# MecatronicaUSB/uw-slam

Hardware: AMD Instinct MI355X
Metric: frame-pair alignments/sec (640x480, 4 pyr lvls) (higher is better)
Workload: dtype f32; 1 GPU; synthetic 640x480 pairs, 4 pyramid levels (0..3), 10 GN iterations/level, no early exit, dense points, u16 depth plane, 1024 pairs in total, 1024 resident on rank 0 (128 distinct), image pyramids of both frames + depth pyramid and gradients of the reference frame + alignment per step; normal_equation_accumulation=f64, weights=identity, tuning=defaults, sampler=nearest, total_pairs=1024, pairs_on_rank0=1024

## Files before the change

uw-slam_amd/csrc/uwt_capi.hip:

```cpp
#include "uwt_ctx.h"

namespace {

constexpr int kGroupsPerThread = 1;

uwt_tuning default_tuning() {
  uwt_tuning t;
  std::memset(&t, 0, sizeof(t));
  t.split = 2;
  t.split_min = 8;
  t.split_min_px = 32LL * 640 * 480;
  t.stream_bytes = 200LL << 20;
  t.tail_update = 1;
  t.target_blocks = 0;
  t.coarse = 1;
  t.coarse_batch_px = kCoarseMaxPixels;
  t.coarse_weighted = 1;
  t.overlap_gradients = 1;
  t.first_poll = 3;
  t.chained = -1;
  t.speculation = 1;
  t.fused_stages = 1;
  t.pyramid_batch = 1;
  t.typed_loads = 1;
// ... 333 lines not shown
  };
  int smax = 1;
  for (int lvl = p.first_level; lvl >= p.last_level; lvl--) {
    int gpb, sl;
    level_slicing(c, lvl, n_pairs, target_blocks, !p.early_exit, gpb, sl);
    smax = std::max(smax, sl);
  }
  if (general && p.weights)
    HIPCHK(c, hipMemsetAsync(c->hist, 0, sizeof(unsigned int) * kHistBins * n_pairs, c->stream));
  bool coarse_lvl[UWT_MAX_LEVELS] = {};
  if (p.accumulate_f64 != 0 && (!general || (p.sampler == 0 && p.weights != 0 && c->tn.coarse_weighted)) && c->tn.coarse_batch_px > 0 &&
      !c->compute_only && !(c->profiling && p.early_exit))
    for (int lvl = p.first_level; lvl >= p.last_level; lvl--)
      coarse_lvl[lvl] = c->lv[lvl].ng <= c->tn.coarse_batch_px;
  auto run_coarse = [&](int base, int cnt, hipStream_t s, int lvl, bool resume) -> int {
    CoarseArgs ca = coarse_args(update_rule(p, general), start.rec(p), InlinePairs{});
    coarse_level(c, ca, 0, lvl);
    ca.n_levels = 1;
    ca.u.pair_base = base;
    ca.state_out = c->state;
    ca.resume = resume ? 1 : 0;
    size_t ev = 0;
    if (c->profiling) {
      int st = prof_begin(c, &ev, lvl, p.max_iters);
      if (st) return st;
    }
    uwt::launch_coarse_level(s, launch_sel(c), ca, cnt, general ? p.weights : 0);
    HIPCHK(c, hipGetLastError());
    if (c->profiling) HIPCHK(c, prof_end(c, ev, s, (long long)cnt * c->lv[lvl].gw * c->lv[lvl].gh, p.max_iters));
    return UWT_OK;
  };
  const bool tickets = c->tn.tail_update >= (parts > 1 ? 1 : 2);
  const bool tail = tickets && !c->compute_only;
  if (tickets) HIPCHK(c, hipMemsetAsync(c->d_tickets, 0, sizeof(unsigned int) * (size_t)n_pairs, c->stream));
  struct Part { int base, cnt; hipStream_t s; ResidualArgs ra; UpdateArgs ua; };
  Part pt[uwt_ctx::kMaxParts];
  const bool window = opt.window && !general && !p.early_exit && p.last_level == 0 && p.first_level >= 1 && !c->profiling &&
                      !c->compute_only;
  struct JoinGuard {
    uwt_ctx* c; int parts; bool joined = false;
    ~JoinGuard() {
      if (joined) return;
      for (int i = 1; i < parts; i++) (void)hipStreamSynchronize(c->part_stream[i]);
    }
  } guard{c, parts};
  if (parts > 1) HIPCHK(c, hipEventRecord(c->ev_fork, c->stream));
  for (int i = 0; i < parts; i++) {
    Part& q = pt[i];
    q.base = (int)((long long)n_pairs * i / parts);
    q.cnt = (int)((long long)n_pairs * (i + 1) / parts) - q.base;
    q.s = i ? c->part_stream[i] : c->stream;
    if (i) HIPCHK(c, hipStreamWaitEvent(q.s, c->ev_fork, 0));
    if (!coarse_lvl[p.first_level]) {
      hipLaunchKernelGGL(k_init_state, dim3((q.cnt + tb - 1) / tb), dim3(tb), 0, q.s, c->state + q.base, q.cnt, start.rec(p, q.base),
                         nullptr);
      HIPCHK(c, hipGetLastError());
    }
  }
  for (int lvl = p.first_level; lvl >= p.last_level; lvl--) {
    for (int i = 0; i < parts; i++) {
      Part& q = pt[i];
      HIPCHK(c, wait_level(c, q.s, level_ready, lvl));
      if (coarse_lvl[lvl]) {
        int st = run_coarse(q.base, q.cnt, q.s, lvl, lvl != p.first_level);
        if (st) return st;
        if (window && lvl == 1) HIPCHK(c, hipEventRecord(c->ev_window[i], q.s));
        continue;
      }
      q.ra = residual_args(c, lvl);
      q.ua = update_args(c, lvl, general);
      q.ra.pair_base = q.ua.pair_base = q.base;
      q.ra.stream_planes = streams(lvl);
      level_slicing(c, lvl, n_pairs, target_blocks, !p.early_exit, q.ra.groups_per_block, q.ra.slices);
      q.ua.slices = q.ra.slices;
      const size_t shift = (size_t)q.base * (size_t)(smax - q.ra.slices) * kRecWords;
      q.ra.partials = c->partials + shift;
      q.ua.partials = c->partials + shift;
    }
    if (coarse_lvl[lvl]) continue;
    LatePoll late(c->tn.first_poll);
    bool level_done = false;
    for (int k = 0; k < p.max_iters && !level_done; k++)
      for (int i = 0; i < parts; i++) {
        Part& q = pt[i];
        size_t ev = 0;
        if (c->profiling) {
          int st = prof_begin(c, &ev, lvl);
          if (st) return st;
          q.ra.probe = 1;
          c->prof_slices = q.ra.slices;
          c->prof_pairs = q.cnt;
          c->prof_records = c->partials;
        }
        q.ua.k = k;
        int st = late.arm(c, q.s, p.early_exit != 0, k, p.max_iters, &q.ua.active);
        if (st) return st;
        if (tail) arm_tail(c, q.ra, q.ua);
        st = general ? launch_general(c, q.s, q.ra, q.cnt, false) : launch_residual(c, q.s, q.ra, q.cnt, false);
        if (st) return st;
        if (c->profiling) HIPCHK(c, prof_end(c, ev, q.s, (long long)q.cnt * c->lv[lvl].gw * c->lv[lvl].gh));
        if (!tail) {
          hipLaunchKernelGGL(k_gn_update, dim3(q.cnt), dim3(kUpdateBlock), 0, q.s, q.ua);
          HIPCHK(c, hipGetLastError());
        }
        st = late.look(c, q.s, &level_done);
        if (st) return st;
        if (level_done) break;
      }
    for (int i = 0; i < parts; i++) {
      hipLaunchKernelGGL(k_level_end, dim3((pt[i].cnt + tb - 1) / tb), dim3(tb), 0, pt[i].s, c->state + pt[i].base, pt[i].cnt, lvl,
                         start.rec(p));
      HIPCHK(c, hipGetLastError());
      if (window && lvl == 1) HIPCHK(c, hipEventRecord(c->ev_window[i], pt[i].s));
    }
  }
  for (int i = 0; i < parts; i++) {
    hipLaunchKernelGGL(k_write_out, dim3((pt[i].cnt + tb - 1) / tb), dim3(tb), 0, pt[i].s, c->state + pt[i].base, pt[i].cnt,
                       d_poses + 7 * (size_t)pt[i].base, d_stats ? d_stats + pt[i].base : nullptr);
    HIPCHK(c, hipGetLastError());
    if (window && parts > 1 && i == 0) HIPCHK(c, hipEventRecord(c->ev_first_end, pt[0].s));
    if (i) {
      HIPCHK(c, hipEventRecord(c->ev_join[i], pt[i].s));
      HIPCHK(c, hipStreamWaitEvent(c->stream, c->ev_join[i], 0));
    }
  }
  guard.joined = true;
  if (window) c->win_parts = parts;
  return UWT_OK;
}

int dep_note(uwt_ctx* c, uwt_ctx::SlotDep* ring, int& next, bool& dropped, hipStream_t on, int first, int n) {
  uwt_ctx::SlotDep& d = ring[next];
  if (d.used) dropped = true;
  d.first = first; d.n = n; d.used = true;
  HIPCHK(c, hipEventRecord(d.ev, on));
  next = (next + 1) % uwt_ctx::kDeps;
  return UWT_OK;
}

}

namespace uwt {

int first_failure(uwt_ctx* c, const char* what, const uwt_stats* stats, int n) {
  for (int i = 0; i < n; i++)
    if (stats[i].status != UWT_OK)
      return fail(c, UWT_ERR_PAIR_FAILED, std::string(what) + ": at least one pair failed, first status: " +
                                              uwt_status_string(stats[i].status));
  return UWT_OK;
}

int seed_options(uwt_ctx* c, const char* what, const uwt_seed_options* sopt, Start* out) {
  *out = Start();
  if (!sopt) return UWT_OK;
  if (sopt->handoff < 0 || sopt->handoff > 1)
    return fail(c, UWT_ERR_INVALID_ARG, std::string(what) + ": uwt_seed_options: handoff outside 0..1");
  for (int32_t r : sopt->reserved)
    if (r) return fail(c, UWT_ERR_INVALID_ARG, std::string(what) + ": uwt_seed_options: reserved word not zero");
  out->keep = sopt->handoff;
  return UWT_OK;
// ... 590 lines not shown
  for (hipEvent_t e : {c->ev_fork, c->ev_pyramids, c->ev_side_done, c->ev_entry, c->ev_first_end}) drop(e);
  for (int i = 0; i < uwt_ctx::kDeps; i++) { drop(c->busy[i].ev); drop(c->fresh[i].ev); }
  for (hipStream_t s : c->part_stream)
    if (s) (void)hipStreamDestroy(s);
  for (hipStream_t s : {c->side, c->copy, c->stream})
    if (s) (void)hipStreamDestroy(s);
  delete c;
  return UWT_OK;
}

int uwt_get_params(const uwt_ctx* c, uwt_params* out) {
  if (!c || !out) return UWT_ERR_INVALID_ARG;
  *out = c->p;
  return UWT_OK;
}

int uwt_get_tuning(const uwt_ctx* c, uwt_tuning* out) {
  if (!c || !out) return UWT_ERR_INVALID_ARG;
  *out = c->tn;
  return UWT_OK;
}

int uwt_set_tuning(uwt_ctx* c, const uwt_tuning* t) {
  if (!c || !t) return UWT_ERR_INVALID_ARG;
  if (t->split < 1 || t->split > uwt_ctx::kMaxParts || t->split_min < 1 || t->split_min_px < 1 || t->stream_bytes < 0 ||
      t->tail_update < 0 || t->tail_update > 2 || t->target_blocks < 0 || t->target_blocks > (1 << 20) || t->coarse_batch_px < 0 ||
      t->coarse_batch_px > (1 << 24) || t->first_poll < 1 || t->first_poll > (1 << 20) || t->chained < -1 || t->chained > 1)
    return fail(c, UWT_ERR_INVALID_ARG, "uwt_set_tuning: value out of range");
  (void)hipSetDevice(c->p.device);
  close_window(c);
  HIPCHK(c, hipStreamSynchronize(c->stream));
  HIPCHK(c, hipStreamSynchronize(c->side));
  c->tn = *t;
  c->spec_budget = c->spec_calm = 0;
  for (int32_t* b : {&c->tn.coarse, &c->tn.coarse_weighted, &c->tn.speculation, &c->tn.fused_stages, &c->tn.pyramid_batch, &c->tn.typed_loads})
    *b = *b != 0;
  if (c->tn.overlap_gradients < 0 || c->tn.overlap_gradients > 3) c->tn.overlap_gradients = 1;
  std::memset(c->tn.reserved, 0, sizeof(c->tn.reserved));
  return UWT_OK;
}

int uwt_update_params(uwt_ctx* c, const uwt_params* p) {
  if (!c || !p) return UWT_ERR_INVALID_ARG;
  const uwt_params& o = c->p;
  if (p->width != o.width || p->height != o.height || p->fx != o.fx || p->fy != o.fy || p->cx != o.cx || p->cy != o.cy ||
      p->n_levels != o.n_levels || p->has_depth != o.has_depth || p->max_frames != o.max_frames ||
      p->max_pairs != o.max_pairs || p->device != o.device || p->depth_scale != o.depth_scale)
    return fail(c, UWT_ERR_INVALID_ARG, "uwt_update_params: geometry / capacity fields differ from the context's");
  if (p->first_level >= p->n_levels || p->last_level < 0 || p->last_level > p->first_level || p->max_iters < 1 ||
      p->sampler < 0 || p->sampler > 1 || p->weights < 0 || p->weights > 2 || (p->sampler == 1 && p->weights == 1) ||
      (p->arith != UWT_ARITH_OPENCV && p->arith != UWT_ARITH_LEGACY))
    return fail(c, UWT_ERR_INVALID_ARG, "uwt_update_params: bad solver constants");
  (void)hipSetDevice(o.device);
  close_window(c);
  HIPCHK(c, hipStreamSynchronize(c->stream));
  if (p->sampler || p->weights) {
    const int st = ensure_general_buffers(c);
    if (st) return st;
  }
  c->p = *p;
  c->spec_budget = c->spec_calm = 0;
  return UWT_OK;
}

int uwt_level_info(const uwt_ctx* c, int32_t lvl, uwt_level* out) {
  if (!c || !out || lvl < 0 || lvl >= c->p.n_levels) return UWT_ERR_INVALID_ARG;
  *out = c->info[lvl];
  return UWT_OK;
}

int uwt_set_frame(uwt_ctx* c, int32_t slot, const uint8_t* gray, size_t row_stride, const uint16_t* depth,
                  size_t depth_row_stride) {
  if (c) (void)hipSetDevice(c->p.device);
  if (!c || !gray || !slot_range_ok(c, slot, 1)) return fail(c, UWT_ERR_INVALID_ARG, "uwt_set_frame: bad slot/pointer");
  const int w = c->p.width;
  if (row_stride < (size_t)w) return fail(c, UWT_ERR_INVALID_ARG, "uwt_set_frame: row stride < width");
  int st0 = compute_begin(c, slot, 1);
  if (st0) return st0;
  if (c->p.has_depth && (!depth || depth_row_stride < (size_t)w * 2)) return fail(c, UWT_ERR_INVALID_ARG, "uwt_set_frame: depth required");
  if ((st0 = copy_strided_frame_in(c, c->img[0], gray, 1, row_stride, slot, c->stream))) return st0;
  if (c->p.has_depth && (st0 = copy_strided_frame_in(c, c->depth[0], depth, 2, depth_row_stride, slot, c->stream))) return st0;
  HIPCHK(c, hipStreamSynchronize(c->stream));
  return UWT_OK;
}

int uwt_host_alloc(size_t bytes, void** out) {
  if (!out || !bytes) return UWT_ERR_INVALID_ARG;
  *out = nullptr;
  return hipHostMalloc(out, bytes) == hipSuccess ? UWT_OK : UWT_ERR_HIP;
}

int uwt_host_free(void* p) { return (!p || hipHostFree(p) == hipSuccess) ? UWT_OK : UWT_ERR_HIP; }

// ... 204 lines not shown
    const int base = c->tn.first_poll + 1;
    if (c->h_small->cut == 0) {
      if (c->spec_budget > base && ++c->spec_calm >= uwt_ctx::kSpecCalm) { c->spec_budget = std::max(base, c->spec_budget / 2); c->spec_calm = 0; }
      break;
    }
    c->spec_calm = 0;
    c->spec_budget = std::min(c->p.max_iters, 2 * std::max(c->spec_budget, base));
    if (attempt == 1) opt.speculate = false;
  }
  if (c->profiling) {
    st = prof_collect(c);
    if (st) return st;
  }
  if (stats_out) std::copy(tmp.begin(), tmp.end(), stats_out);
  return first_failure(c, what, tmp.data(), n_pairs);
}

int uwt_estimate_pose_batch(uwt_ctx* c, int32_t n_pairs, const int32_t* ref_slots, const int32_t* tgt_slots,
                            float* poses_out, uwt_stats* stats_out) {
  return estimate_pose_batch(c, "uwt_estimate_pose_batch", n_pairs, ref_slots, tgt_slots, poses_out, stats_out, nullptr, nullptr);
}

int uwt_default_seed_options(uwt_seed_options* o) {
  if (!o) return UWT_ERR_INVALID_ARG;
  std::memset(o, 0, sizeof(*o));
  return UWT_OK;
}

int uwt_estimate_pose_batch_seeded(uwt_ctx* c, int32_t n_pairs, const int32_t* ref_slots, const int32_t* tgt_slots,
                                   float* poses_out, uwt_stats* stats_out, const float* seeds, const uwt_seed_options* sopt) {
  return estimate_pose_batch(c, "uwt_estimate_pose_batch_seeded", n_pairs, ref_slots, tgt_slots, poses_out, stats_out, seeds, sopt);
}

static int track_batch_enqueue(uwt_ctx* c, int32_t first_slot, int32_t n_frames, int32_t grad_refs_only, int32_t n_pairs,
                               const int32_t* ref_slots, const int32_t* tgt_slots, float* d_poses_out, uwt_stats* d_stats_out,
                               const Start& start = Start()) {
  if (c) (void)hipSetDevice(c->p.device);
  if (!c) return fail(c, UWT_ERR_INVALID_ARG, "uwt_track_batch_async: bad argument");
  const bool had_window = c->win_open;
  const int win_parts = c->win_parts;
  close_window(c);
  c->win_parts = 0;
  if (!d_poses_out || !slot_range_ok(c, first_slot, n_frames))
    return fail(c, UWT_ERR_INVALID_ARG, "uwt_track_batch_async: bad argument");
  int st = seeds_clear_of(c, "uwt_track_batch_seeded_async", start.d_seeds, n_pairs, d_poses_out, d_stats_out);
  if (st) return st;
  const int og = c->tn.overlap_gradients;
  const bool overlap = og != 0 && !c->profiling && (n_pairs >= 768 || og == 3);
  const bool early = had_window && overlap && og != 2;
  st = check_pair_lists_range(c, n_pairs, ref_slots, tgt_slots);
  if (st) return st;
  struct SideGuard {
    uwt_ctx* c; bool armed = false;
    ~SideGuard() { if (armed) (void)hipStreamSynchronize(c->side); }
  } side_guard{c};
  if (early) {
    HIPCHK(c, hipEventRecord(c->ev_entry, c->stream));
    side_guard.armed = true;
    for (int i = 0; i < win_parts; i++) HIPCHK(c, hipStreamWaitEvent(c->side, c->ev_window[i], 0));
    if (win_parts > 1) HIPCHK(c, hipStreamWaitEvent(c->side, c->ev_first_end, 0));
  }
  st = send_pairs(c, n_pairs, ref_slots, tgt_slots, early);
  if (st) return st;
  int lo = first_slot, hi = first_slot + n_frames;
  for (int i = 0; i < n_pairs; i++) {
    lo = std::min(lo, std::min(ref_slots[i], tgt_slots[i]));
    hi = std::max(hi, std::max(ref_slots[i], tgt_slots[i]) + 1);
  }
  c->dep_first = lo;
// ... 171 lines not shown
```

uw-slam_amd/csrc/uwt_capi_tables.hip:

```cpp
#include "uwt_ctx.h"
#include "uwt_track.h"

extern "C" {

namespace {

int check_keypoints(uwt_ctx* c, const char* what, const float* kp, int n) {
  const float w = (float)c->lv[0].gw, h = (float)c->lv[0].gh;
  for (int i = 0; i < std::min(n, kPatchMaxKeypoints); i++)
    if (!inside_level0(kp[2 * i], kp[2 * i + 1], w, h))
      return fail(c, UWT_ERR_INVALID_ARG, std::string(what) + ": key point outside the image");
  return UWT_OK;
}

struct CandidatesLayout {
  int bands;
  size_t o_sums, o_mag, o_cells, o_off;
};
CandidatesLayout candidates_work_layout(Carve& cv, const LevelK& L, int n) {
  CandidatesLayout o;
  const int col_blocks = (L.gw + kBlock - 1) / kBlock;
  o.bands = std::max(1, std::min(L.gh / 8, 512 / std::max(1, col_blocks * n)));
  const size_t m = (size_t)L.gw * o.bands * n;
  o.o_sums = cv.take<unsigned long long>((size_t)n);
// ... 192 lines not shown
  HIPCHK(c, hipEventRecord(c->ev_feat[stage], c->stream));
  return enqueue_patch_producer(c, n, d_slots);
}

int table_options(uwt_ctx* c, const char* what, const uwt_table_options* opt, uwt_table_options* out) {
  std::memset(out, 0, sizeof(*out));
  if (!opt) return UWT_OK;
  if (opt->weights < 0 || opt->weights > 2 || opt->sampler < 0 || opt->sampler > 1)
    return fail(c, UWT_ERR_INVALID_ARG, std::string(what) + ": uwt_table_options: weights outside 0..2 or sampler outside 0..1");
  for (int32_t r : opt->reserved)
    if (r) return fail(c, UWT_ERR_INVALID_ARG, std::string(what) + ": uwt_table_options: reserved word not zero");
  *out = *opt;
  return UWT_OK;
}
constexpr uwt_table_options kIdentityTables = {};

struct TableLevel {
  TableArgs ta;
  int slices;
};

int enqueue_table_estimate(uwt_ctx* c, int n_pairs, const uwt_params& q, const TableLevel* lv, uint32_t* recs, bool polls,
                           const uwt_table_options& opt, float* d_poses, StatsOut* d_stats, const Start& start = Start()) {
  const int tb = 128, blocks = (n_pairs + tb - 1) / tb;
  const bool general = opt.weights || opt.sampler;
  if (opt.weights) {
    int st = ensure_general_buffers(c);
    if (st) return st;
    HIPCHK(c, hipMemsetAsync(c->hist, 0, sizeof(unsigned int) * kHistBins * (size_t)n_pairs, c->stream));
  }
  const GeneralArgs ga = {opt.sampler, opt.weights, q.gain, c->hist, c->scale};
  hipLaunchKernelGGL(k_init_state, dim3(blocks), dim3(tb), 0, c->stream, c->state, n_pairs, start.rec(q), start.d_gate);
  HIPCHK(c, hipGetLastError());
  HIPCHK(c, hipMemsetAsync(c->d_tickets, 0, sizeof(unsigned int) * (size_t)n_pairs, c->stream));
  for (int lvl = q.first_level; lvl >= q.last_level; lvl--) {
    ResidualArgs ra = residual_args(c, lvl, q);
    ra.slices = lv[lvl].slices;
    ra.partials = recs;
    UpdateArgs ua = update_args(c, lvl, q, general);
    ua.partials = recs;
    ua.slices = ra.slices;
    LatePoll late(c->tn.first_poll);
    for (int k = 0; k < q.max_iters; k++) {
      ua.k = k;
      int st = late.arm(c, c->stream, polls, k, q.max_iters, &ua.active);
      if (st) return st;
      arm_tail(c, ra, ua);
      if (general) uwt::launch_table_general(c->stream, launch_sel(c), ra, lv[lvl].ta, ga, n_pairs);
      else uwt::launch_table_eval(c->stream, launch_sel(c), ra, lv[lvl].ta, n_pairs);
      HIPCHK(c, hipGetLastError());
      bool none_left = false;
      st = late.look(c, c->stream, &none_left);
      if (st) return st;
      if (none_left) break;
    }
    hipLaunchKernelGGL(k_level_end, dim3(blocks), dim3(tb), 0, c->stream, c->state, n_pairs, lvl, start.rec(q));
    HIPCHK(c, hipGetLastError());
  }
  hipLaunchKernelGGL(k_write_out, dim3(blocks), dim3(tb), 0, c->stream, c->state, n_pairs, d_poses, d_stats);
  HIPCHK(c, hipGetLastError());
  return UWT_OK;
}

int features_enqueue(uwt_ctx* c, const char* what, int n_pairs, const int32_t* ref_slots, const int32_t* tgt_slots, const float* kp,
                     const int32_t* n_kp, const uwt_table_options* opt_or_null, float* d_poses, StatsOut* d_stats,
                     const Start& start = Start()) {
// ... 322 lines not shown
```

uw-slam_amd/csrc/uwt_ctx.h:

```cpp
#pragma once

#include "../../include/uwt.h"

#include <hip/hip_runtime.h>

#include <cmath>
#include <cstdio>
#include <cstring>
#include <algorithm>
#include <initializer_list>
#include <new>
#include <string>
#include <vector>

#include "uwt_launch.h"

static_assert(sizeof(uwt::StatsOut) == sizeof(uwt_stats), "uwt_stats layout");

namespace uwt {

struct GuardGap { long long at; size_t bytes; int array; };
constexpr unsigned char kGuardPattern = 0xC7;
struct Carve;
struct DevBuf {
// ... 55 lines not shown
  uint8_t* img[UWT_MAX_LEVELS] = {};
  uint16_t* depth[UWT_MAX_LEVELS] = {};
  int16_t* gx[UWT_MAX_LEVELS] = {};
  int16_t* gy[UWT_MAX_LEVELS] = {};
  PairState* state = nullptr;
  int* d_ref = nullptr;
  int* d_tgt = nullptr;
  int* d_pair_set[2] = {};
  int pair_set = 0;
  static constexpr int kPairStages = 4;
  int* h_pairs = nullptr;
  hipEvent_t ev_pairs[kPairStages] = {};
  int pair_stage[2] = {0, 1};
  int n_pairs_cached[2] = {0, 0};
  int pair_stage_last = 1;
  struct SlotDep { int first = 0, n = 0; hipEvent_t ev = nullptr; bool used = false; };
  static constexpr int kDeps = 8;
  hipStream_t copy = nullptr;
  SlotDep busy[kDeps], fresh[kDeps];
  int busy_next = 0, fresh_next = 0;
  long long ticket_seq = 0;
  long long busy_seq[kDeps] = {};
  bool busy_dropped = false, fresh_dropped = false;
  uint32_t* partials = nullptr;
  uint32_t* partials2 = nullptr;
  PairState* state2 = nullptr;
  size_t partial_records = 0;
  float* d_poses = nullptr;
  StatsOut* d_stats = nullptr;
  unsigned int* hist = nullptr;
  PairScale* scale = nullptr;
  int* d_active = nullptr;
  unsigned int* d_tickets = nullptr;
  int* h_active = nullptr;
  size_t guard_bytes = 0;
  DevBuf scratch;
  float4* feat_tab = nullptr;
  int* feat_cnt = nullptr;
  float2* feat_kp = nullptr;
  int* feat_nkp = nullptr;
  uint32_t* feat_recs = nullptr;
  float* h_feat = nullptr;
  hipEvent_t ev_feat[kPairStages] = {};
  int feat_stage = 0;
  DevBuf cand_tab, cand_cnt, cand_work, cand_recs;
  DevBuf match_desc, match_cnt, match_part, match_out;
  DevBuf ransac_buf;
  int* ransac_need = nullptr;
  std::vector<int> ransac_need_host;
  std::vector<unsigned char> ransac_row_done;
  double ransac_need_confidence = 0.0;
  int ransac_need_hypotheses = 0;
  DevBuf surf_buf;
  DevBuf orb_buf, orb_pat;
  int8_t orb_pattern[1024] = {};
  int orb_pattern_state = 0;
  DevBuf track_buf;
  DevBuf warp_buf;
  DevBuf cloud_buf;
  int* h_cloud = nullptr;
  hipEvent_t ev_cloud[kPairStages] = {};
  int cloud_stage = 0;
  DevBuf stage[2];
  bool profiling = false;
  int spec_budget = 0;
  int spec_calm = 0;
// ... 113 lines not shown
```

uw-slam_amd/csrc/uwt_kernels.h:

```cpp
#pragma once

#include <hip/hip_runtime.h>
#include <stdint.h>

#include <type_traits>

#include "uwt_math.h"

namespace uwt {

constexpr int kBlock = 256;
constexpr int kAccFloats = 27;
constexpr int kRecWords = 64;
constexpr int kMaxSlices = 160;

constexpr int kArithOpenCV = 0, kArithLegacy = 1;

struct LevelK {
  int pitch;
  int iw, ih;
  int gw, gh;
  int n;
  int ng;
  float fx, fy, cx, cy, invfx, invfy;
// ... 986 lines not shown
  for (int pass = 0; pass < 2; pass++) {
    for (int i = threadIdx.x; i < 256; i += blockDim.x) hist[i] = 0;
    __syncthreads();
    for (int i = threadIdx.x; i < n; i += blockDim.x) {
      const float v = pass == 0 ? r[i] : fabsf(r[i] - s_med);
      int q = (int)rintf(v);
      q = q < 0 ? 0 : (q > 255 ? 255 : q);
      atomicAdd(&hist[q], 1u);
    }
    __syncthreads();
    if (threadIdx.x == 0) {
      const float med = median_of_hist();
      if (pass == 0) s_med = med; else s_mad = 1.4826f * med;
    }
    __syncthreads();
  }
  if (threadIdx.x == 0) { out_stats[0] = s_med; out_stats[1] = s_mad; }
  if (!w) return;
  float mad = s_mad;
  if (mad == 0.0f) mad = 1.0f;
  const float inv_mad = (float)(1.0 / (double)mad);
  for (int i = threadIdx.x; i < n; i += blockDim.x) w[i] = robust_weight(kind, r[i], inv_mad);
}

struct UpdateRule {
  int max_iters;
  int early_exit;
  float epsilon;
  float gain;
  int general;
  int legacy_solve;
};

struct TailUpdate {
  unsigned int* tickets;
  PairState* state;
  int* active;
  int on;
  int k;
  UpdateRule rule;
};

struct ResidualArgs {
  const uint8_t* img;
  const int16_t* gx;
  const int16_t* gy;
  const uint16_t* depth;
  const int* ref_slots;
  const int* tgt_slots;
  const PairState* state;
  Pose pose;
  LevelK L;
  float zf, af;
  int groups_per_block;
  int slices;
  int pair_base;
  uint32_t* partials;
  const PairScale* scale;
  float gain;
  float* dumpJ;
  float* dumpR;
  uint8_t* dumpV;
  float* dumpW;
  int typed_loads;
  int stream_planes;
  int probe;
  TailUpdate tail;
};

struct CoreOverride {
  int groups_per_block;
  uint32_t* rec;
  const PairScale* scale = nullptr;
// ... 539 lines not shown
      pe += kBlock * VEC;
      if (it + 1 < iters) {
        body(rgB, 1, rg);
        pe += kBlock * VEC;
      }
    }
    wait_planes_typed<DEPTH>(rg);
    wait_planes_typed<DEPTH>(rgB);
  } else {
    for (int it = 0; it < iters; it++, g += kBlock) body(rg, 1, rg);
  }
  const uint32_t n_valid = (threadIdx.x & 63) == 0 ? n_valid_wave : 0u;
  uint32_t* out_rec = ov ? ov->rec : a.partials + ((size_t)pair * a.slices + slice) * kRecWords;
  constexpr bool R2D = MASKED && !GENERAL;
  const bool coherent = !ov && a.tail.on != 0;
  if constexpr (EXT_LDS != 0 && R2D) block_reduce_store_at<AccT, false, EXT_LDS, double>(lds, acc, r2d, n_valid, out_rec, err);
  else if constexpr (EXT_LDS != 0) block_reduce_store_at<AccT, GENERAL, EXT_LDS>(lds, acc, sum_r2, n_valid, out_rec, err);
  else if constexpr (TABLE) {
    __syncthreads();
    block_reduce_store_at<AccT, true>(tlds, acc, sum_r2, n_valid, out_rec, err, coherent);
  } else if constexpr (TYPED) {
    __syncthreads();
    block_reduce_store_at<AccT, false, kBatchPass, double>(tlds, acc, r2d, n_valid, out_rec, err, coherent);
  } else if constexpr (R2D) block_reduce_store<AccT, false, double>(acc, r2d, n_valid, out_rec, err, coherent);
  else block_reduce_store<AccT, GENERAL>(acc, sum_r2, n_valid, out_rec, err, coherent);
  if (a_probe && threadIdx.x == 0) {
    uint32_t* rec = a.partials + ((size_t)pair * a.slices + slice) * kRecWords;
    rec[60] = (uint32_t)(__builtin_amdgcn_s_memtime() - s_probe[0]);
    rec[61] = (uint32_t)(__builtin_amdgcn_s_memrealtime() - s_probe[1]);
  }
}

__device__ __forceinline__ void tail_update_wave(const ResidualArgs& a, int pair);

template <int AR, int VEC, bool DEPTH, bool UNIT_FACTORS, bool DUMP, typename AccT, bool SQUARE = false, int SAMPLER = 0, int WEIGHTS = 0,
          bool COMPUTE_ONLY = false, int STREAM = 0, bool RAGGED = false>
__global__ __launch_bounds__(kBlock) void k_residual(const ResidualArgs a) {
  const int pair = (int)blockIdx.y + a.pair_base;
  const bool live = residual_block<AR, VEC, DEPTH, UNIT_FACTORS, DUMP, AccT, SQUARE, SAMPLER, WEIGHTS, COMPUTE_ONLY, STREAM, RAGGED>(a, pair, (int)blockIdx.x);
  if constexpr (!COMPUTE_ONLY && !DUMP) {
    if (a.tail.on && live && threadIdx.x < 64) tail_update_wave(a, pair);
  }
}

template <int AR, int VEC, bool DEPTH, bool UNIT_FACTORS, bool DUMP, typename AccT, bool SQUARE = false, int SAMPLER = 0, int WEIGHTS = 0,
          int STREAM = 0, bool RAGGED = false>
__global__ __launch_bounds__(kBlock) __attribute__((amdgpu_waves_per_eu(4, 4))) void k_residual_w4(const ResidualArgs a) {
  const int pair = (int)blockIdx.y + a.pair_base;
  const bool live = residual_block<AR, VEC, DEPTH, UNIT_FACTORS, DUMP, AccT, SQUARE, SAMPLER, WEIGHTS, false, STREAM, RAGGED>(a, pair, (int)blockIdx.x);
  if constexpr (!DUMP) {
    if (a.tail.on && live && threadIdx.x < 64) tail_update_wave(a, pair);
  }
}

struct GeneralArgs {
  int sampler;
  int weights;
  float gain;
  unsigned int* hist;
  PairScale* scale;
};

__device__ __forceinline__ int first_crossing(const unsigned int v[8], float m, int lane) {
  unsigned int tot = 0;
#pragma unroll
  for (int k = 0; k < 8; k++) tot += v[k];
  unsigned int inc = tot;
#pragma unroll
  for (int d = 1; d < 64; d <<= 1) {
    const unsigned int up = __shfl_up(inc, d, 64);
    if (lane >= d) inc += up;
  }
  unsigned int cum = inc - tot;
  int idx = 0x7fffffff;
#pragma unroll
  for (int k = 0; k < 8; k++) {
    cum += v[k];
    if (idx == 0x7fffffff && (float)cum > m) idx = lane * 8 + k;
  }
#pragma unroll
  for (int d = 32; d > 0; d >>= 1) idx = min(idx, __shfl_xor(idx, d, 64));
  return idx;
}

// ... 273 lines not shown
  bool update = true;
  if (n == 0) {
    st.status = 2;
    st.level_done = 1;
    update = false;
  } else {
    const float inv_n = (float)(1.0 / (double)n);
    const float error = a.general ? (float)((double)inv_n * sums[kAccFloats])
                                  : (float)((double)inv_n * (double)sr2);
    st.error = error;
    if (a.early_exit &&
        (error >= st.last_error || k == a.max_iters - 1 || fabsf(error - st.last_error) < a.epsilon)) {
      st.level_done = 1;
      update = false;
    } else {
      st.last_error = error;
    }
  }
  if (update) {
    float b[6], delta[6];
#pragma unroll
    for (int i = 0; i < 6; i++)
      b[i] = a.general ? (float)(-sums[21 + i]) : (float)(-((double)a.gain * sums[21 + i]));
    solve_delta_wave(sums, b, delta, a.legacy_solve != 0);
    Pose d, np;
    se3_exp_wave(delta, d);
    se3_mul(st.pose, d, np);
    st.pose = np;
    if (active && lane == 0) atomicAdd(active, 1);
  }
}

constexpr int kTailRounds = 4;
__device__ __forceinline__ void tail_fold_wave(const ResidualArgs& a, int pair, int stride, int count) {
  __shared__ __attribute__((aligned(16))) double t_sums[kAccFloats + 1];
  __shared__ long long t_isums[2];
  const int lane = (int)threadIdx.x;
  unsigned int ticket = 0;
  if (lane == 0) ticket = __hip_atomic_fetch_add(a.tail.tickets + pair, 1u, __ATOMIC_RELAXED, __HIP_MEMORY_SCOPE_AGENT);
  ticket = (unsigned int)__builtin_amdgcn_readfirstlane((int)ticket);
  if (ticket != (unsigned int)count - 1u) return;
  if (lane == 0) __hip_atomic_store(a.tail.tickets + pair, 0u, __ATOMIC_RELAXED, __HIP_MEMORY_SCOPE_AGENT);
  const int slot = lane & 31, half = lane >> 5;
  const unsigned long long* g8 = reinterpret_cast<const unsigned long long*>(a.partials + (size_t)pair * stride * kRecWords) + slot;
  double cs[4] = {0.0, 0.0, 0.0, 0.0};
  long long is[4] = {0, 0, 0, 0};
  for (int q0 = 0; q0 < count; q0 += 8 * kTailRounds) {
    unsigned long long v[kTailRounds][4];
#pragma unroll
    for (int r = 0; r < kTailRounds; r++)
#pragma unroll
      for (int j = 0; j < 4; j++) {
        const int q = q0 + 8 * r + half + 2 * j;
        v[r][j] = q < count ? __hip_atomic_load(g8 + (size_t)q * (kRecWords / 2), __ATOMIC_RELAXED, __HIP_MEMORY_SCOPE_AGENT) : 0ull;
      }
#pragma unroll
    for (int r = 0; r < kTailRounds; r++)
#pragma unroll
      for (int j = 0; j < 4; j++) {
        cs[j] += __longlong_as_double((long long)v[r][j]);
        is[j] += (long long)(slot == 27 ? (v[r][j] & 0xffffffffull) : v[r][j]);
      }
  }
  double fs = 0.0;
  long long ls = 0;
#pragma unroll
  for (int j = 0; j < 4; j++) {
    const double of = __shfl_xor(cs[j], 32);
    const long long oi = __shfl_xor(is[j], 32);
    if (j == 0) { fs = cs[0]; ls = is[0]; } else { fs += cs[j]; ls += is[j]; }
    fs += of;
    ls += oi;
  }
  if (lane < 32) {
    if (lane < kAccFloats) t_sums[lane] = fs;
    else if (lane == 27) t_isums[0] = (long long)(uint32_t)ls;
    else if (lane == 28) t_isums[1] = ls;
    else if (lane == 29) t_sums[kAccFloats] = a.tail.rule.general ? fs : 0.0;
  }
  __builtin_amdgcn_wave_barrier();
  PairState st = a.tail.state[pair];
  update_solve_wave(a.tail.rule, a.tail.k, a.tail.active, st, t_sums, t_isums, lane);
  if (lane == 0) a.tail.state[pair] = st;
}

__device__ __forceinline__ void tail_update_wave(const ResidualArgs& a, int pair) { tail_fold_wave(a, pair, a.slices, a.slices); }

__device__ __forceinline__ PairState update_compute(const UpdateArgs& a, const uint32_t* __restrict__ recs, const PairState* __restrict__ st_in,
                                                    unsigned char* __restrict__ lds, bool count_active) {
  const int tid = (int)thread_here(), lane = tid & 63;
  double(*part_f)[32] = reinterpret_cast<double(*)[32]>(lds);
  long long(*part_i)[32] = reinterpret_cast<long long(*)[32]>(lds + 8 * 32 * 8);
  double* sums = reinterpret_cast<double*>(lds + 2 * 8 * 32 * 8);
  long long* isums = reinterpret_cast<long long*>(sums + kAccFloats + 1);
  PairState* s_state = reinterpret_cast<PairState*>(isums + 2);
  const int slot = tid & 31, part = tid >> 5;
  const unsigned long long* g8 = reinterpret_cast<const unsigned long long*>(recs) + slot;
  unsigned long long v[kFoldBatch];
#pragma unroll
  for (int u = 0; u < kFoldBatch; u++) {
    const int q = part + 8 * u;
    v[u] = q < a.slices ? g8[(size_t)q * (kRecWords / 2)] : 0ull;
  }
  PairState st = *st_in;
  const bool live = !(st.level_done || st.status);
  if (live) {
    double cs = 0.0;
    long long is = 0;
    for (int q0 = part;;) {
#pragma unroll
      for (int u = 0; u < kFoldBatch; u++) {
        cs += __longlong_as_double((long long)v[u]);
        is += (long long)(slot == 27 ? (v[u] & 0xffffffffull) : v[u]);
      }
      q0 += 8 * kFoldBatch;
      if (q0 >= a.slices) break;
#pragma unroll
      for (int u = 0; u < kFoldBatch; u++) {
        const int q = q0 + 8 * u;
// ... 5 lines not shown
    __syncthreads();
    if (tid < 32) {
      double fs = part_f[0][tid];
      long long ls = part_i[0][tid];
#pragma unroll
      for (int q = 1; q < 8; q++) {
        fs += part_f[q][tid];
        ls += part_i[q][tid];
      }
      if (tid < kAccFloats) sums[tid] = fs;
      else if (tid == 27) isums[0] = (long long)(uint32_t)ls;
      else if (tid == 28) isums[1] = ls;
      else if (tid == 29) sums[kAccFloats] = a.rule.general ? fs : 0.0;
    }
  }
  __builtin_amdgcn_wave_barrier();
  if (tid < 64) {
    if (live) update_solve_wave(a.rule, a.k, count_active ? a.active : nullptr, st, sums, isums, lane);
    if (lane == 0) *s_state = st;
  }
  __syncthreads();
  return *s_state;
}

static __global__ __launch_bounds__(kUpdateBlock) void k_gn_update(const UpdateArgs a) {
  __shared__ __attribute__((aligned(16))) unsigned char lds[kUpdateLdsBytes];
  const int pair = (int)blockIdx.x + a.pair_base;
  const PairState st = update_compute(a, a.partials + (size_t)pair * a.slices * kRecWords, &a.state[pair], lds, true);
  if (threadIdx.x == 0) a.state[pair] = st;
}

constexpr int kHandoffKeep = 2;
constexpr int kStatusBadSeed = 1;

struct StartRec {
  int scale_t;
  const float* seeds;
  float initial_error;
};

__device__ __forceinline__ PairState fresh_state(const Pose& pose, float initial_error) {
  PairState st;
  st.pose = pose;
  st.last_error = initial_error;
  st.error = 0.f;
  st.level_done = 0;
  st.status = 0;
  st.iters = 0;
  st.n_valid = 0;
  return st;
}

__device__ __forceinline__ PairState first_state(const StartRec& s, int pair, bool seeded = true) {
  Pose id;
  pose_identity(id);
  PairState st = fresh_state(id, s.initial_error);
  if (s.seeds && seeded) {
    float v[7];
    bool finite = true;
#pragma unroll
    for (int k = 0; k < 7; k++) {
      v[k] = s.seeds[7 * (size_t)pair + k];
      finite = finite && (__float_as_uint(v[k]) & 0x7f800000u) != 0x7f800000u;
    }
    if (finite) {
#pragma unroll
      for (int k = 0; k < 4; k++) st.pose.q[k] = v[k];
#pragma unroll
      for (int k = 0; k < 3; k++) st.pose.t[k] = v[4 + k];
    } else {
      st.status = kStatusBadSeed;
    }
// ... 212 lines not shown
            unsigned int t = 0;
            if (b < 511) {
              const uint4 lo = *reinterpret_cast<const uint4*>(&h[b * kHistRep]), hi = *reinterpret_cast<const uint4*>(&h[b * kHistRep + 4]);
              t = lo.x + lo.y + lo.z + lo.w + hi.x + hi.y + hi.z + hi.w;
            }
            mine[q] = t;
          }
          const PairScale sc = wave_scale(mine, h_scratch, WEIGHTS == kWeightsTukeyRef, lane);
          if (lane == 0) s_scale = sc;
        }
        __syncthreads();
        residual_core<AR, VEC, DEPTH, PLAIN, false, double, PLAIN, 0, WEIGHTS, false, 0, 0, RAGGED>(a, pair, 0, st.pose, nullptr, nullptr, ref_slot, tgt_slot, &ov);
        __syncthreads();
        u.k = k;
        st = update_compute(u, rec, &cur, ulds, false);
        if (st.level_done || st.status) break;
      }
    }
    level_end(st, ca.level_id[li], ca.start);
  }
  if (threadIdx.x == 0) ca.state_out[pair] = st;
}

struct StatsOut { int status, iterations, n_valid; float error; };

__device__ __forceinline__ void write_result(const PairState& st, int pair, float* __restrict__ poses, StatsOut* __restrict__ stats) {
  for (int k = 0; k < 4; k++) poses[7 * pair + k] = st.pose.q[k];
  for (int k = 0; k < 3; k++) poses[7 * pair + 4 + k] = st.pose.t[k];
  if (stats) {
    StatsOut o;
    o.status = st.status; o.iterations = st.iters; o.n_valid = st.n_valid; o.error = st.error;
    stats[pair] = o;
  }
}

static __global__ __launch_bounds__(kUpdateBlock) void k_finish(const IterArgs ia, float* __restrict__ poses, StatsOut* __restrict__ stats) {
  __shared__ __attribute__((aligned(16))) unsigned char lds[kUpdateLdsBytes];
  const int pair = (int)blockIdx.x + ia.u.pair_base;
  const PairState st = iterate_state(ia, pair, lds, true);
  if (threadIdx.x) return;
  ia.state_out[pair] = st;
  write_result(st, pair, poses, stats);
}

static __global__ void k_set_pose(PairState* state, Pose pose, float initial_error) {
  if (threadIdx.x || blockIdx.x) return;
  state[0] = fresh_state(pose, initial_error);
}

static __global__ void k_init_state(PairState* state, int n, const StartRec start, const int* __restrict__ gate) {
  const int i = blockIdx.x * blockDim.x + threadIdx.x;
  if (i >= n) return;
  state[i] = first_state(start, i, !(gate && gate[i] == 0));
}

static __global__ void k_level_end(PairState* state, int n, int lvl, const StartRec start) {
  const int i = blockIdx.x * blockDim.x + threadIdx.x;
  if (i >= n) return;
  PairState st = state[i];
  level_end(st, lvl, start);
  state[i] = st;
}

static __global__ void k_write_out(const PairState* state, int n, float* poses, StatsOut* stats) {
  const int i = blockIdx.x * blockDim.x + threadIdx.x;
  if (i >= n) return;
// ... 621 lines not shown
```

Before: 71260 alignments/s.

## Fold level-end and write-out into last residual tail update; skip redundant ticket memsets

On the final Gauss-Newton iteration of each level, the tail-update wave inside the residual kernel now applies the level-end transition and, on the last level, writes poses and stats. This removes the separate k_level_end and k_write_out launches. Idle pairs get the same treatment from block 0 of the residual grid. The per-call ticket memset is also skipped when the tickets are known to be clean, with the clean flag reset on errors, tuning or parameter changes, and in the general path. The cost is more host-side state that must stay correct, and some extra work on the tail wave.

Result: no change. 71250 alignments/s (-0.0%).

```diff
diff --git a/uw-slam_amd/csrc/uwt_capi.hip b/uw-slam_amd/csrc/uwt_capi.hip
--- a/uw-slam_amd/csrc/uwt_capi.hip
+++ b/uw-slam_amd/csrc/uwt_capi.hip
@@ -389,7 +389,11 @@
   };
   const bool tickets = c->tn.tail_update >= (parts > 1 ? 1 : 2);
   const bool tail = tickets && !c->compute_only;
-  if (tickets) HIPCHK(c, hipMemsetAsync(c->d_tickets, 0, sizeof(unsigned int) * (size_t)n_pairs, c->stream));
+  const bool tail_ends = tail && !general && !p.early_exit && !c->profiling;
+  if (tickets) {
+    if (!c->tickets_clean) HIPCHK(c, hipMemsetAsync(c->d_tickets, 0, sizeof(unsigned int) * (size_t)c->p.max_pairs, c->stream));
+    c->tickets_clean = false;
+  }
   struct Part { int base, cnt; hipStream_t s; ResidualArgs ra; UpdateArgs ua; };
   Part pt[uwt_ctx::kMaxParts];
   const bool window = opt.window && !general && !p.early_exit && p.last_level == 0 && p.first_level >= 1 && !c->profiling &&
@@ -453,6 +457,13 @@
         int st = late.arm(c, q.s, p.early_exit != 0, k, p.max_iters, &q.ua.active);
         if (st) return st;
         if (tail) arm_tail(c, q.ra, q.ua);
+        if (tail_ends && k == p.max_iters - 1) {
+          q.ra.tail.end = lvl == p.last_level ? 2 : 1;
+          q.ra.tail.lvl = lvl;
+          q.ra.tail.start = start.rec(p);
+          q.ra.tail.poses = d_poses;
+          q.ra.tail.stats = d_stats;
+        }
         st = general ? launch_general(c, q.s, q.ra, q.cnt, false) : launch_residual(c, q.s, q.ra, q.cnt, false);
         if (st) return st;
         if (c->profiling) HIPCHK(c, prof_end(c, ev, q.s, (long long)q.cnt * c->lv[lvl].gw * c->lv[lvl].gh));
@@ -465,16 +476,21 @@
         if (level_done) break;
       }
     for (int i = 0; i < parts; i++) {
-      hipLaunchKernelGGL(k_level_end, dim3((pt[i].cnt + tb - 1) / tb), dim3(tb), 0, pt[i].s, c->state + pt[i].base, pt[i].cnt, lvl,
-                         start.rec(p));
+      if (!tail_ends) {
+        hipLaunchKernelGGL(k_level_end, dim3((pt[i].cnt + tb - 1) / tb), dim3(tb), 0, pt[i].s, c->state + pt[i].base, pt[i].cnt, lvl,
+                           start.rec(p));
+        HIPCHK(c, hipGetLastError());
+      }
+      if (window && lvl == 1) HIPCHK(c, hipEventRecord(c->ev_window[i], pt[i].s));
+    }
+  }
+  const bool wrote = tail_ends && !coarse_lvl[p.last_level];
+  for (int i = 0; i < parts; i++) {
+    if (!wrote) {
+      hipLaunchKernelGGL(k_write_out, dim3((pt[i].cnt + tb - 1) / tb), dim3(tb), 0, pt[i].s, c->state + pt[i].base, pt[i].cnt,
+                         d_poses + 7 * (size_t)pt[i].base, d_stats ? d_stats + pt[i].base : nullptr);
       HIPCHK(c, hipGetLastError());
-      if (window && lvl == 1) HIPCHK(c, hipEventRecord(c->ev_window[i], pt[i].s));
-    }
-  }
-  for (int i = 0; i < parts; i++) {
-    hipLaunchKernelGGL(k_write_out, dim3((pt[i].cnt + tb - 1) / tb), dim3(tb), 0, pt[i].s, c->state + pt[i].base, pt[i].cnt,
-                       d_poses + 7 * (size_t)pt[i].base, d_stats ? d_stats + pt[i].base : nullptr);
-    HIPCHK(c, hipGetLastError());
+    }
     if (window && parts > 1 && i == 0) HIPCHK(c, hipEventRecord(c->ev_first_end, pt[0].s));
     if (i) {
       HIPCHK(c, hipEventRecord(c->ev_join[i], pt[i].s));
@@ -483,6 +499,7 @@
   }
   guard.joined = true;
   if (window) c->win_parts = parts;
+  if (tickets) c->tickets_clean = true;
   return UWT_OK;
 }
 
@@ -1139,6 +1156,7 @@
   HIPCHK(c, hipStreamSynchronize(c->stream));
   HIPCHK(c, hipStreamSynchronize(c->side));
   c->tn = *t;
+  c->tickets_clean = false;
   c->spec_budget = c->spec_calm = 0;
   for (int32_t* b : {&c->tn.coarse, &c->tn.coarse_weighted, &c->tn.speculation, &c->tn.fused_stages, &c->tn.pyramid_batch, &c->tn.typed_loads})
     *b = *b != 0;
@@ -1166,6 +1184,7 @@
     if (st) return st;
   }
   c->p = *p;
+  c->tickets_clean = false;
   c->spec_budget = c->spec_calm = 0;
   return UWT_OK;
 }
@@ -1436,9 +1455,22 @@
   return estimate_pose_batch(c, "uwt_estimate_pose_batch_seeded", n_pairs, ref_slots, tgt_slots, poses_out, stats_out, seeds, sopt);
 }
 
+static int track_batch_enqueue_checked(uwt_ctx* c, int32_t first_slot, int32_t n_frames, int32_t grad_refs_only, int32_t n_pairs,
+                                       const int32_t* ref_slots, const int32_t* tgt_slots, float* d_poses_out, uwt_stats* d_stats_out,
+                                       const Start& start);
+
 static int track_batch_enqueue(uwt_ctx* c, int32_t first_slot, int32_t n_frames, int32_t grad_refs_only, int32_t n_pairs,
                                const int32_t* ref_slots, const int32_t* tgt_slots, float* d_poses_out, uwt_stats* d_stats_out,
                                const Start& start = Start()) {
+  const int st = track_batch_enqueue_checked(c, first_slot, n_frames, grad_refs_only, n_pairs, ref_slots, tgt_slots, d_poses_out,
+                                             d_stats_out, start);
+  if (st && c) c->tickets_clean = false;
+  return st;
+}
+
+static int track_batch_enqueue_checked(uwt_ctx* c, int32_t first_slot, int32_t n_frames, int32_t grad_refs_only, int32_t n_pairs,
+                                       const int32_t* ref_slots, const int32_t* tgt_slots, float* d_poses_out, uwt_stats* d_stats_out,
+                                       const Start& start) {
   if (c) (void)hipSetDevice(c->p.device);
   if (!c) return fail(c, UWT_ERR_INVALID_ARG, "uwt_track_batch_async: bad argument");
   const bool had_window = c->win_open;
diff --git a/uw-slam_amd/csrc/uwt_capi_tables.hip b/uw-slam_amd/csrc/uwt_capi_tables.hip
--- a/uw-slam_amd/csrc/uwt_capi_tables.hip
+++ b/uw-slam_amd/csrc/uwt_capi_tables.hip
@@ -248,6 +248,7 @@
   const GeneralArgs ga = {opt.sampler, opt.weights, q.gain, c->hist, c->scale};
   hipLaunchKernelGGL(k_init_state, dim3(blocks), dim3(tb), 0, c->stream, c->state, n_pairs, start.rec(q), start.d_gate);
   HIPCHK(c, hipGetLastError());
+  c->tickets_clean = false;
   HIPCHK(c, hipMemsetAsync(c->d_tickets, 0, sizeof(unsigned int) * (size_t)n_pairs, c->stream));
   for (int lvl = q.first_level; lvl >= q.last_level; lvl--) {
     ResidualArgs ra = residual_args(c, lvl, q);
diff --git a/uw-slam_amd/csrc/uwt_ctx.h b/uw-slam_amd/csrc/uwt_ctx.h
--- a/uw-slam_amd/csrc/uwt_ctx.h
+++ b/uw-slam_amd/csrc/uwt_ctx.h
@@ -111,6 +111,7 @@
   PairScale* scale = nullptr;
   int* d_active = nullptr;
   unsigned int* d_tickets = nullptr;
+  bool tickets_clean = true;
   int* h_active = nullptr;
   size_t guard_bytes = 0;
   DevBuf scratch;
diff --git a/uw-slam_amd/csrc/uwt_kernels.h b/uw-slam_amd/csrc/uwt_kernels.h
--- a/uw-slam_amd/csrc/uwt_kernels.h
+++ b/uw-slam_amd/csrc/uwt_kernels.h
@@ -1042,13 +1042,25 @@
   int legacy_solve;
 };
 
+struct StartRec {
+  int scale_t;
+  const float* seeds;
+  float initial_error;
+};
+struct StatsOut;
+
 struct TailUpdate {
   unsigned int* tickets;
   PairState* state;
   int* active;
   int on;
   int k;
+  int end;
+  int lvl;
   UpdateRule rule;
+  StartRec start;
+  float* poses;
+  StatsOut* stats;
 };
 
 struct ResidualArgs {
@@ -1654,6 +1666,12 @@
 }
 
 __device__ __forceinline__ void tail_update_wave(const ResidualArgs& a, int pair);
+__device__ __forceinline__ void tail_end_idle(const TailUpdate& t, int pair);
+
+__device__ __forceinline__ void residual_tail(const ResidualArgs& a, int pair, bool live) {
+  if (live) tail_update_wave(a, pair);
+  else if (a.tail.end && blockIdx.x == 0 && threadIdx.x == 0) tail_end_idle(a.tail, pair);
+}
 
 template <int AR, int VEC, bool DEPTH, bool UNIT_FACTORS, bool DUMP, typename AccT, bool SQUARE = false, int SAMPLER = 0, int WEIGHTS = 0,
           bool COMPUTE_ONLY = false, int STREAM = 0, bool RAGGED = false>
@@ -1661,7 +1679,7 @@
   const int pair = (int)blockIdx.y + a.pair_base;
   const bool live = residual_block<AR, VEC, DEPTH, UNIT_FACTORS, DUMP, AccT, SQUARE, SAMPLER, WEIGHTS, COMPUTE_ONLY, STREAM, RAGGED>(a, pair, (int)blockIdx.x);
   if constexpr (!COMPUTE_ONLY && !DUMP) {
-    if (a.tail.on && live && threadIdx.x < 64) tail_update_wave(a, pair);
+    if (a.tail.on && threadIdx.x < 64) residual_tail(a, pair, live);
   }
 }
 
@@ -1671,7 +1689,7 @@
   const int pair = (int)blockIdx.y + a.pair_base;
   const bool live = residual_block<AR, VEC, DEPTH, UNIT_FACTORS, DUMP, AccT, SQUARE, SAMPLER, WEIGHTS, false, STREAM, RAGGED>(a, pair, (int)blockIdx.x);
   if constexpr (!DUMP) {
-    if (a.tail.on && live && threadIdx.x < 64) tail_update_wave(a, pair);
+    if (a.tail.on && threadIdx.x < 64) residual_tail(a, pair, live);
   }
 }
 
@@ -2011,7 +2029,9 @@
 }
 
 constexpr int kTailRounds = 4;
-__device__ __forceinline__ void tail_fold_wave(const ResidualArgs& a, int pair, int stride, int count) {
+__device__ __forceinline__ void level_end(PairState& st, int lvl, const StartRec& s);
+__device__ __forceinline__ void write_result(const PairState& st, int pair, float* __restrict__ poses, StatsOut* __restrict__ stats);
+__device__ __forceinline__ void tail_fold_wave(const ResidualArgs& a, int pair, int stride, int count, bool ends = false) {
   __shared__ __attribute__((aligned(16))) double t_sums[kAccFloats + 1];
   __shared__ long long t_isums[2];
   const int lane = (int)threadIdx.x;
@@ -2060,10 +2080,14 @@
   __builtin_amdgcn_wave_barrier();
   PairState st = a.tail.state[pair];
   update_solve_wave(a.tail.rule, a.tail.k, a.tail.active, st, t_sums, t_isums, lane);
-  if (lane == 0) a.tail.state[pair] = st;
-}
-
-__device__ __forceinline__ void tail_update_wave(const ResidualArgs& a, int pair) { tail_fold_wave(a, pair, a.slices, a.slices); }
+  if (lane == 0) {
+    if (ends && a.tail.end) level_end(st, a.tail.lvl, a.tail.start);
+    a.tail.state[pair] = st;
+    if (ends && a.tail.end == 2) write_result(st, pair, a.tail.poses, a.tail.stats);
+  }
+}
+
+__device__ __forceinline__ void tail_update_wave(const ResidualArgs& a, int pair) { tail_fold_wave(a, pair, a.slices, a.slices, true); }
 
 __device__ __forceinline__ PairState update_compute(const UpdateArgs& a, const uint32_t* __restrict__ recs, const PairState* __restrict__ st_in,
                                                     unsigned char* __restrict__ lds, bool count_active) {
@@ -2135,12 +2159,6 @@
 
 constexpr int kHandoffKeep = 2;
 constexpr int kStatusBadSeed = 1;
-
-struct StartRec {
-  int scale_t;
-  const float* seeds;
-  float initial_error;
-};
 
 __device__ __forceinline__ PairState fresh_state(const Pose& pose, float initial_error) {
   PairState st;
@@ -2419,6 +2437,13 @@
     o.status = st.status; o.iterations = st.iters; o.n_valid = st.n_valid; o.error = st.error;
     stats[pair] = o;
   }
+}
+
+__device__ __forceinline__ void tail_end_idle(const TailUpdate& t, int pair) {
+  PairState st = t.state[pair];
+  level_end(st, t.lvl, t.start);
+  t.state[pair] = st;
+  if (t.end == 2) write_result(st, pair, t.poses, t.stats);
 }
 
 static __global__ __launch_bounds__(kUpdateBlock) void k_finish(const IterArgs ia, float* __restrict__ poses, StatsOut* __restrict__ stats) {
```
